# yeyupiaoling/PPASR

Hardware: AMD Instinct MI355X
Metric: audio-seconds/s (RTF^-1) Conformer-streaming fbank, batch32 per GPU, ctc_greedy (higher is better)
Workload: dtype f32; 1 GPU; configs[1]: Conformer streaming (configs/conformer.yml), fbank-80, 32 x 10 s utterances per GPU, V=4233, ctc_greedy, features resident in HBM -> token ids + scores on device; global_batch=32, frames=1000, decoder=ctc_greedy, parallelism=utterance-dp1, pipelined=False, gemm=f32

## Files before the change

### ppasr_amd/csrc/front_fused.hip

```cpp
#include <utility>

#include "conformer_kernels.h"
#include "launch.h"

namespace ppasr {

namespace {
constexpr int kGroupRow[5] = {2, 0, 1, 4, 3};
constexpr int kTapCol[5] = {2, 0, 1, 4, 3};
constexpr int kFactor[5] = {2, 0, 1, 3, 1};
constexpr int quad_slab(int t) { return 4 * kFactor[t / 5] + kFactor[t % 5]; }
constexpr int quad_target(int t) {
  const int g = t / 5, k = t % 5;
  if (g == 0) return k == 0 ? 4 : k <= 2 ? 5 : 4;
  const int a = (g == 1 || g == 2) ? 0 : 2;
  return k == 0 ? (a == 0 ? 5 : 4) : k <= 2 ? a : a + 1;
}
constexpr int quad_fold_src(int t) {
  return t == 1 || t == 5 || t == 21 || t == 23 ? 4 : t == 3 || t == 11 || t == 13 ? 5 : -1;
}
constexpr int quad_fold_mask(int t) {
  return t == 1 ? 0xf : t == 3 ? 0x5 : t == 5 ? 0xa : t == 11 ? 0x2 : t == 13 ? 0x1 : t == 21 ? 0x8 : t == 23 ? 0x4 : 0;
}
constexpr bool quad_fold_clear(int t) { return t == 1 || t == 3 || t == 5 || t == 13 || t == 23; }
static_assert(quad_target(0) == 4 && quad_target(2) == 5 && quad_target(10) == 5 && quad_target(12) == 0 &&
                  quad_target(14) == 1 && quad_target(20) == 4 && quad_target(22) == 2 && quad_target(24) == 3,
              "chunk targets");

template <typename Fn, int... I>
__device__ __forceinline__ void static_for(std::integer_sequence<int, I...>, Fn&& fn) {
  (fn(std::integral_constant<int, I>{}), ...);
}

__host__ __device__ inline int quad_xs_stride(int F, int Q) { return F > 8 * Q + 3 ? F : 8 * Q + 3; }
}

template <bool FROM_Y1>
__device__ __forceinline__ void conv2_quad_body(const float* __restrict__ src, const FrontW& fw, float* __restrict__ out,
                                                int T, int F, int Tp, int F2, int M, int m0, const PadSkip& ps,
                                                const int* __restrict__ tile_tab) {
  constexpr int BP = 32, KC = 128, LD = KC + 4, G = KC / 8, NL = 2, N_CHUNKS = 25;
  constexpr int SLOT = BP * LD;
  const int P = (Tp + 1) >> 1;
  const int Q = (F2 + 1) >> 1;
  int r0 = m0 + blockIdx.x * BP, Mlim = M;
  if (tile_tab) {
    const int t = blockIdx.x, nb = tile_tab[0];
    const int* pre = tile_tab + 1;
    if (t >= pre[nb]) return;
    int lo = 0, hi = nb;
    while (hi - lo > 1) {
      const int mid = (lo + hi) >> 1;
      if (pre[mid] <= t) lo = mid;
      else hi = mid;
    }
    const int S = ps.Tp * ps.unit;
    r0 = lo * S + (t - pre[lo]) * BP;
    Mlim = min(M, (lo + 1) * S);
  } else if (pad_block_skippable(ps, r0, BP, M)) {
    return;
  }
  extern __shared__ __attribute__((aligned(16))) float smem[];
  float* const slot0 = smem;
  float* const slot1 = smem + SLOT;
  f32x4* const y2s = reinterpret_cast<f32x4*>(smem + 2 * SLOT);
  float* const w1s = smem + 2 * SLOT + 5 * NL * 4 * kThreads;
  float* const xs = w1s + 10 * 256;
  const int tid = threadIdx.x, lane = lane_id(), wave = wave_id();
  constexpr int tile_stride = 2 * 16 * G * 64;
  const f32x4* wbase = fw.conv2_wp + (size_t)wave * tile_stride;
  auto seg = [&](int h, int slab) { return wbase + (size_t)(16 * h + slab) * G * 64; };
  BRing<1> ring;
  ring_prime(ring, seg(0, quad_slab(0)), 0);
  const int c4 = tid & 31, rbase = tid >> 5;
  const int bp0 = r0 / Q;
  const int FX = quad_xs_stride(F, Q);
  uint32_t pb = 0;
  int yrow[FROM_Y1 ? NL : 1], yp4[FROM_Y1 ? NL : 1], yq4[FROM_Y1 ? NL : 1];
  if constexpr (!FROM_Y1) {
    for (int idx = tid; idx < 10 * 256; idx += kThreads) w1s[idx] = idx < 9 * 256 ? fw.conv1_w[idx] : fw.conv1_b[idx - 9 * 256];
    const int nbp = (min(r0 + BP, Mlim) - 1) / Q - bp0 + 1;
    for (int idx = tid; idx < nbp * 11 * FX; idx += kThreads) {
      const int fr_row = idx / FX, f = idx - fr_row * FX;
      const int bpl = fr_row / 11, fr = fr_row - 11 * bpl;
      const int bp = bp0 + bpl, b = bp / P, p = bp - b * P;
      const int t = min(8 * p + fr, T - 1);
      xs[idx] = f < F ? (src[((size_t)b * T + t) * F + f] - fw.cmvn_mean[f]) * fw.cmvn_istd[f] : 0.f;
    }
#pragma unroll
    for (int i = 0; i < NL; ++i) {
      const int m = r0 + rbase + 16 * i;
      const int bp = m / Q, q = m - bp * Q;
      const uint32_t v = m < Mlim ? (uint32_t)((bp - bp0) * 11 * FX + 8 * q) : 0xffffu;
      pb |= v << (16 * i);
    }
  } else {
#pragma unroll
    for (int i = 0; i < NL; ++i) {
      const int m = r0 + rbase + 16 * i;
      const int bp = m / Q, q = m - bp * Q, b = bp / P, p = bp - b * P;
      yrow[i] = b * T + 4 * p;
      yp4[i] = 4 * p;
      yq4[i] = m < Mlim ? 4 * q : -1;
    }
  }
  auto pbase = [&](int i) { return (int)((pb >> (16 * i)) & 0xffffu); };
  const int lds_off0 = rbase * LD + 4 * c4;
  float xv[9];
  f32x4 wv[3], bv, ya, yv;
  auto y1_step = [&](int i, int h, int r, int c, int step) {
    const int cc = h * 128 + 4 * c4;
    if constexpr (!FROM_Y1) {
      if (step == 0) {
        const int o = pbase(i);
        const float* p = xs + (o == 0xffff ? 0 : o) + 2 * r * FX + 2 * c;
#pragma unroll
        for (int ii = 0; ii < 3; ++ii)
#pragma unroll
          for (int jj = 0; jj < 3; ++jj) xv[ii * 3 + jj] = p[ii * FX + jj];
        ya = f32x4{0.f, 0.f, 0.f, 0.f};
      } else {
#pragma unroll
        for (int j = 3 * (step - 1); j < 3 * step; ++j)
#pragma unroll
          for (int e = 0; e < 4; ++e) ya[e] = fmaf(wv[j % 3][e], xv[j], ya[e]);
        if (step == 3) {
          ya += bv;
#pragma unroll
          for (int e = 0; e < 4; ++e) ya[e] = pbase(i) != 0xffff ? fmaxf(ya[e], 0.f) : 0.f;
        }
      }
      if (step < 3) {
#pragma unroll
        for (int j = 0; j < 3; ++j) wv[j] = *reinterpret_cast<const f32x4*>(w1s + (3 * step + j) * 256 + cc);
        if (step == 2) bv = *reinterpret_cast<const f32x4*>(w1s + 9 * 256 + cc);
      }
    } else {
      if (step == 0) {
        yv = f32x4{0.f, 0.f, 0.f, 0.f};
        if (yq4[i] >= 0 && yp4[i] + r < T && yq4[i] + c < F)
          yv = *reinterpret_cast<const f32x4*>(src + ((size_t)(yrow[i] + r) * F + yq4[i] + c) * 256 + cc);
      } else if (step == 3) {
        ya = yv;
      }
    }
  };
  auto put = [&](float* buf, int i, const f32x4& v) { *reinterpret_cast<f32x4*>(buf + lds_off0 + i * 16 * LD) = v; };
  auto y2row = [&](int c, int i) -> f32x4& { return y2s[(c * NL + i) * kThreads + tid]; };
  f32x4 z2[NL];
  auto build = [&](auto nc, int g, int h, float* buf) {
    constexpr int n = decltype(nc)::value, grp = n / 5, k = n % 5, r = kGroupRow[grp], c = kTapCol[k];
    const int i = g >> 2, step = g & 3;
    y1_step(i, h, r, c, step);
    if (step != 3) return;
    f32x4 v = ya;
    if constexpr (grp == 0) y2row(c, i) = ya;
    if constexpr (grp == 1 || grp == 3) v = ya - y2row(c, i);
    if constexpr (k == 0) {
      z2[i] = v;
      put(buf, i, v);
    } else if constexpr (k == 1 || k == 3) {
      put(buf, i, v - z2[i]);
    } else {
      put(buf, i, v);
    }
  };
  f32x16 acc[6][1][1];
#pragma unroll
  for (int a = 0; a < 6; ++a) acc_zero(acc[a]);
  auto fold = [&](auto tc, int g) {
    constexpr int t = decltype(tc)::value, fs = quad_fold_src(t), mask = quad_fold_mask(t);
    if constexpr (fs >= 0) {
      const int j = g - 4 * NL;
      int seen = 0;
#pragma unroll
      for (int o = 0; o < 4; ++o) {
        if (!((mask >> o) & 1)) continue;
        if (seen++ == j) {
#pragma unroll
          for (int e = 0; e < 16; ++e) asm volatile("v_add_f32 %0, %0, %1" : "+v"(acc[o][0][0][e]) : "v"(acc[fs][0][0][e]));
        }
      }
      if (quad_fold_clear(t) && j == 4) acc_zero(acc[fs]);
    }
  };
  __syncthreads();
#pragma unroll
  for (int g = 0; g < 4 * NL; ++g) {
    build(std::integral_constant<int, 0>{}, g, 0, slot0);
    __builtin_amdgcn_sched_barrier(0);
  }
  __syncthreads();
  for (int h = 0; h < 2; ++h) {
    asm volatile("" : "+s"(wbase));
    if constexpr (!FROM_Y1) {
      asm volatile("" : "+v"(pb));
    } else {
#pragma unroll
      for (int i = 0; i < NL; ++i) asm volatile("" : "+v"(yrow[i]), "+v"(yp4[i]), "+v"(yq4[i]));
    }
    static_for(std::make_integer_sequence<int, N_CHUNKS>{}, [&](auto tc) {
      constexpr int t = decltype(tc)::value;
      float* const cur = ((t + h) & 1) ? slot1 : slot0;
      float* const nxb = ((t + h) & 1) ? slot0 : slot1;
      const f32x4* nseg = t + 1 < N_CHUNKS ? seg(h, quad_slab(t + 1)) : (h == 0 ? seg(1, quad_slab(0)) : nullptr);
      auto side = [&](int g) {
        if (g < 4 * NL) {
          if constexpr (t + 1 < N_CHUNKS) build(std::integral_constant<int, t + 1>{}, g, h, nxb);
          else if (h == 0) build(std::integral_constant<int, 0>{}, g, 1, nxb);
        } else {
          fold(tc, g);
        }
      };
      rb_gemm<1, 1, G, kPF, decltype(side)>(cur, LD, seg(h, quad_slab(t)), 0, nseg, 0, ring, acc[quad_target(t)], side);
      __syncthreads();
    });
  }
  const int col = wave * 32 + (lane & 31);
  const float b2 = fw.conv2_b[col];
#pragma unroll
  for (int r = 0; r < 16; ++r) {
    const int m = r0 + acc_row(r, lane);
    if (m >= Mlim) continue;
    const int bp = m / Q, q = m - bp * Q, b = bp / P, t0 = 2 * (bp - b * P), f0 = 2 * q;
    float* o = out + ((size_t)(b * Tp + t0) * F2 + f0) * 256 + col;
    const bool f1 = f0 + 1 < F2, t1 = t0 + 1 < Tp;
    o[0] = fmaxf(acc[0][0][0][r] + b2, 0.f);
    if (f1) o[256] = fmaxf(acc[1][0][0][r] + b2, 0.f);
    if (t1) o[(size_t)F2 * 256] = fmaxf(acc[2][0][0][r] + b2, 0.f);
    if (t1 && f1) o[(size_t)F2 * 256 + 256] = fmaxf(acc[3][0][0][r] + b2, 0.f);
  }
}

__global__ __launch_bounds__(kThreads) void k_conv12(const float* __restrict__ feats, FrontW fw, float* __restrict__ out,
                                                     int T, int F, int Tp, int F2, int M, int m0, PadSkip ps,
                                                     const int* __restrict__ tile_tab) {
  conv2_quad_body<false>(feats, fw, out, T, F, Tp, F2, M, m0, ps, tile_tab);
}
__global__ __launch_bounds__(kThreads) void k_conv2_pair(const float* __restrict__ y1, FrontW fw, float* __restrict__ out,
                                                         int T1, int F1, int Tp, int F2, int M, int m0, PadSkip ps,
                                                         const int* __restrict__ tile_tab) {
  conv2_quad_body<true>(y1, fw, out, T1, F1, Tp, F2, M, m0, ps, tile_tab);
}

static int quad_tile_pairs(int Q) { return 31 / Q + 2; }
static size_t quad_lds(bool fused, int F, int F2) {
  const int Q = (F2 + 1) / 2;
  return ((size_t)2 * 32 * 132 + (size_t)5 * 2 * 4 * 512 + (fused ? (size_t)10 * 256 + (size_t)quad_tile_pairs(Q) * 11 * quad_xs_stride(F, Q) : 0)) *
         sizeof(float);
}
bool conv2_quad_supported(const FrontW& fw) { return fw.conv2_wp && fw.conv2_k == 3 && fw.conv2_s == 2; }
bool conv12_supported(const FrontW& fw, int F, int F2) {
  const int Q = (F2 + 1) / 2;
  return conv2_quad_supported(fw) && F2 >= 1 && quad_lds(true, F, F2) <= 160 * 1024 &&
         (size_t)quad_tile_pairs(Q) * 11 * quad_xs_stride(F, Q) < 0xffff;
}

void launch_tile_prefix(const PadSkip& ps, int B, int BM, int* tab, hipStream_t st);

static void launch_quad(bool fused, const float* src, const FrontW& fw, float* y2, int B, int T, int F, int Tp, int F2,
                        hipStream_t st, const PadSkip& ps_frames, int* tile_scratch) {
  const int P = (Tp + 1) / 2, Q = (F2 + 1) / 2;
  PadSkip ps = ps_frames;
  ps.Tp = P;
  ps.mul = 2 * ps_frames.mul;
  ps.slack = (ps_frames.slack + 1) / 2;
  ps.unit = Q;
  const int M = B * P * Q;
  const int* no_tab = nullptr;
#define QUAD(GRID, TAB)                                                                                                  \
  do {                                                                                                                 \
    if (fused)                                                                                                         \
      PPASR_LAUNCH(k_conv12, dim3(GRID), dim3(kThreads), quad_lds(true, F, F2), st, src, fw, y2, T, F, Tp, F2, M, 0, ps, \
                   TAB);                                                                                               \
    else                                                                                                               \
      PPASR_LAUNCH(k_conv2_pair, dim3(GRID), dim3(kThreads), quad_lds(false, F, F2), st, src, fw, y2, T, F, Tp, F2, M, 0, \
                   ps, TAB);                                                                                           \
  } while (0)
  if (ps.lens && tile_scratch) {
    launch_tile_prefix(ps, B, 32, tile_scratch, st);
    QUAD(B * ((P * Q + 31) / 32), (const int*)tile_scratch);
    return;
  }
  QUAD((M + 31) / 32, no_tab);
#undef QUAD
}

void launch_conv12(const float* feats, const FrontW& fw, float* y2, int B, int T, int F, int Tp, int F2, hipStream_t st,
                   const PadSkip& ps_frames, int* tile_scratch) {
  launch_quad(true, feats, fw, y2, B, T, F, Tp, F2, st, ps_frames, tile_scratch);
}
void launch_conv2_quad(const float* y1, const FrontW& fw, float* y2, int B, int T1, int F1, int Tp, int F2, hipStream_t st,
                       const PadSkip& ps_frames, int* tile_scratch) {
  launch_quad(false, y1, fw, y2, B, T1, F1, Tp, F2, st, ps_frames, tile_scratch);
}

hipError_t configure_front_fused_kernels() {
  hipError_t e;
#define SET_LDS(fn)                                                                                              \
  e = hipFuncSetAttribute(reinterpret_cast<const void*>(fn), hipFuncAttributeMaxDynamicSharedMemorySize, 160 * 1024); \
  if (e != hipSuccess) return e;
  SET_LDS(k_conv12);
  SET_LDS(k_conv2_pair);
#undef SET_LDS
  return hipSuccess;
}

}
```

Measured before the change: 58430 audio-s/s.

## Compute conv1 im2col tile with MFMA 32x32x2 instead of scalar FMAs

In the fused front-end conv kernel, the first 3x3 convolution (conv1) on the CMVN-normalized fbank tile was computed with per-thread scalar FMAs. It is now computed by the first four waves using chains of mfma_f32_32x32x2f32. The bias is folded in as a fifth K pair through a constant-one input, with ReLU applied through inline v_max. Precomputed LDS byte offsets replace the packed per-row base, and the out-of-range rows read a zeroed tail region. This moves conv1 arithmetic off the VALU so it can overlap the conv2 GEMM pipeline. In exchange it adds hand-placed s_nop hazard padding and a different lane-to-row mapping that must stay consistent with the LDS layout.

```diff
diff --git a/ppasr_amd/csrc/front_fused.hip b/ppasr_amd/csrc/front_fused.hip
--- a/ppasr_amd/csrc/front_fused.hip
+++ b/ppasr_amd/csrc/front_fused.hip
@@ -30,6 +30,12 @@
 template <typename Fn, int... I>
 __device__ __forceinline__ void static_for(std::integer_sequence<int, I...>, Fn&& fn) {
   (fn(std::integral_constant<int, I>{}), ...);
+}
+
+__device__ __forceinline__ float relu1(float x) {
+  float d;
+  asm("v_max_f32 %0, 0, %1" : "=v"(d) : "v"(x));
+  return d;
 }
 
 __host__ __device__ inline int quad_xs_stride(int F, int Q) { return F > 8 * Q + 3 ? F : 8 * Q + 3; }
@@ -75,8 +81,10 @@
   const int c4 = tid & 31, rbase = tid >> 5;
   const int bp0 = r0 / Q;
   const int FX = quad_xs_stride(F, Q);
-  uint32_t pb = 0;
+  const int hh = lane >> 5;
   int yrow[FROM_Y1 ? NL : 1], yp4[FROM_Y1 ? NL : 1], yq4[FROM_Y1 ? NL : 1];
+  uint32_t xoff[5] = {0, 0, 0, 0, 0};
+  float one = 0.f;
   if constexpr (!FROM_Y1) {
     for (int idx = tid; idx < 10 * 256; idx += kThreads) w1s[idx] = idx < 9 * 256 ? fw.conv1_w[idx] : fw.conv1_b[idx - 9 * 256];
     const int nbp = (min(r0 + BP, Mlim) - 1) / Q - bp0 + 1;
@@ -87,12 +95,17 @@
       const int t = min(8 * p + fr, T - 1);
       xs[idx] = f < F ? (src[((size_t)b * T + t) * F + f] - fw.cmvn_mean[f]) * fw.cmvn_istd[f] : 0.f;
     }
-#pragma unroll
-    for (int i = 0; i < NL; ++i) {
-      const int m = r0 + rbase + 16 * i;
-      const int bp = m / Q, q = m - bp * Q;
-      const uint32_t v = m < Mlim ? (uint32_t)((bp - bp0) * 11 * FX + 8 * q) : 0xffffu;
-      pb |= v << (16 * i);
+    if (r0 + BP > Mlim)
+      for (int idx = tid; idx < 11 * FX; idx += kThreads) xs[nbp * 11 * FX + idx] = 0.f;
+    const int m = r0 + (lane & 31);
+    const int bp = m / Q, q = m - bp * Q;
+    const bool live = m < Mlim;
+    const int base = (int)(xs - smem) + (live ? (bp - bp0) * 11 * FX + 8 * q : nbp * 11 * FX);
+    one = live ? 1.f : 0.f;
+#pragma unroll
+    for (int mm = 0; mm < 5; ++mm) {
+      const int j = min(2 * mm + hh, 8);
+      xoff[mm] = (uint32_t)(base + (j / 3) * FX + j % 3) * 4u;
     }
   } else {
 #pragma unroll
@@ -104,51 +117,22 @@
       yq4[i] = m < Mlim ? 4 * q : -1;
     }
   }
-  auto pbase = [&](int i) { return (int)((pb >> (16 * i)) & 0xffffu); };
   const int lds_off0 = rbase * LD + 4 * c4;
-  float xv[9];
-  f32x4 wv[3], bv, ya, yv;
+  f32x4 ya, yv;
   auto y1_step = [&](int i, int h, int r, int c, int step) {
     const int cc = h * 128 + 4 * c4;
-    if constexpr (!FROM_Y1) {
-      if (step == 0) {
-        const int o = pbase(i);
-        const float* p = xs + (o == 0xffff ? 0 : o) + 2 * r * FX + 2 * c;
-#pragma unroll
-        for (int ii = 0; ii < 3; ++ii)
-#pragma unroll
-          for (int jj = 0; jj < 3; ++jj) xv[ii * 3 + jj] = p[ii * FX + jj];
-        ya = f32x4{0.f, 0.f, 0.f, 0.f};
-      } else {
-#pragma unroll
-        for (int j = 3 * (step - 1); j < 3 * step; ++j)
-#pragma unroll
-          for (int e = 0; e < 4; ++e) ya[e] = fmaf(wv[j % 3][e], xv[j], ya[e]);
-        if (step == 3) {
-          ya += bv;
-#pragma unroll
-          for (int e = 0; e < 4; ++e) ya[e] = pbase(i) != 0xffff ? fmaxf(ya[e], 0.f) : 0.f;
-        }
-      }
-      if (step < 3) {
-#pragma unroll
-        for (int j = 0; j < 3; ++j) wv[j] = *reinterpret_cast<const f32x4*>(w1s + (3 * step + j) * 256 + cc);
-        if (step == 2) bv = *reinterpret_cast<const f32x4*>(w1s + 9 * 256 + cc);
-      }
-    } else {
-      if (step == 0) {
-        yv = f32x4{0.f, 0.f, 0.f, 0.f};
-        if (yq4[i] >= 0 && yp4[i] + r < T && yq4[i] + c < F)
-          yv = *reinterpret_cast<const f32x4*>(src + ((size_t)(yrow[i] + r) * F + yq4[i] + c) * 256 + cc);
-      } else if (step == 3) {
-        ya = yv;
-      }
+    if (step == 0) {
+      yv = f32x4{0.f, 0.f, 0.f, 0.f};
+      if (yq4[i] >= 0 && yp4[i] + r < T && yq4[i] + c < F)
+        yv = *reinterpret_cast<const f32x4*>(src + ((size_t)(yrow[i] + r) * F + yq4[i] + c) * 256 + cc);
+    } else if (step == 3) {
+      ya = yv;
     }
   };
   auto put = [&](float* buf, int i, const f32x4& v) { *reinterpret_cast<f32x4*>(buf + lds_off0 + i * 16 * LD) = v; };
   auto y2row = [&](int c, int i) -> f32x4& { return y2s[(c * NL + i) * kThreads + tid]; };
   f32x4 z2[NL];
-  auto build = [&](auto nc, int g, int h, float* buf) {
+  auto build_twin = [&](auto nc, int g, int h, float* buf) {
     constexpr int n = decltype(nc)::value, grp = n / 5, k = n % 5, r = kGroupRow[grp], c = kTapCol[k];
     const int i = g >> 2, step = g & 3;
     y1_step(i, h, r, c, step);
@@ -165,6 +149,55 @@
       put(buf, i, v);
     }
   };
+  float w1a[5] = {0.f, 0.f, 0.f, 0.f, 0.f};
+  auto load_w1 = [&](int h) {
+    if (wave >= 4) return;
+#pragma unroll
+    for (int mm = 0; mm < 5; ++mm) w1a[mm] = w1s[(2 * mm + hh) * 256 + h * 128 + 32 * wave + (lane & 31)];
+  };
+  float xw[5];
+  f32x16 y1t;
+  f32x4 zc[4], d1v;
+  const int lds_row0 = (lane & 31) * LD + 32 * (wave & 3) + 4 * hh;
+  auto d1row = [&](int c, int qd) -> f32x4& { return y2s[(c * 4 + qd) * 256 + (tid & 255)]; };
+  auto build_mfma = [&](auto nc, int g, float* buf) {
+    constexpr int n = decltype(nc)::value, grp = n / 5, k = n % 5, r = kGroupRow[grp], c = kTapCol[k];
+    if (wave >= 4) return;
+    if (g == 0) {
+      const uint32_t pos = (uint32_t)(2 * r * FX + 2 * c) * 4u;
+#pragma unroll
+      for (int mm = 0; mm < 5; ++mm)
+        xw[mm] = *reinterpret_cast<const float*>(reinterpret_cast<const char*>(smem) + (xoff[mm] + pos));
+    } else if (g == 1 || g == 2) {
+      if (g == 1) {
+        xw[4] = hh ? one : xw[4];
+        const f32x16 zero = {0.f, 0.f, 0.f, 0.f, 0.f, 0.f, 0.f, 0.f, 0.f, 0.f, 0.f, 0.f, 0.f, 0.f, 0.f, 0.f};
+        y1t = __builtin_amdgcn_mfma_f32_32x32x2f32(w1a[0], xw[0], zero, 0, 0, 0);
+        y1t = __builtin_amdgcn_mfma_f32_32x32x2f32(w1a[1], xw[1], y1t, 0, 0, 0);
+        y1t = __builtin_amdgcn_mfma_f32_32x32x2f32(w1a[2], xw[2], y1t, 0, 0, 0);
+      } else {
+        y1t = __builtin_amdgcn_mfma_f32_32x32x2f32(w1a[3], xw[3], y1t, 0, 0, 0);
+        y1t = __builtin_amdgcn_mfma_f32_32x32x2f32(w1a[4], xw[4], y1t, 0, 0, 0);
+      }
+    }
+    if (g >= 4) {
+      const int qd = g - 4;
+      f32x4 v;
+#pragma unroll
+      for (int e = 0; e < 4; ++e) v[e] = relu1(y1t[4 * qd + e]);
+      if constexpr (grp == 0) d1row(c, qd) = v;
+      if constexpr (grp == 1 || grp == 3) v = v - d1v;
+      if constexpr (k == 0) zc[qd] = v;
+      if constexpr (k == 1 || k == 3) v = v - zc[qd];
+      *reinterpret_cast<f32x4*>(buf + lds_row0 + 8 * qd) = v;
+    }
+    if constexpr (grp == 1 || grp == 3)
+      if (g >= 3 && g < 7) d1v = d1row(c, g - 3);
+  };
+  auto build = [&](auto nc, int g, int h, float* buf) {
+    if constexpr (FROM_Y1) build_twin(nc, g, h, buf);
+    else build_mfma(nc, g, buf);
+  };
   f32x16 acc[6][1][1];
 #pragma unroll
   for (int a = 0; a < 6; ++a) acc_zero(acc[a]);
@@ -185,16 +218,20 @@
     }
   };
   __syncthreads();
+  if constexpr (!FROM_Y1) load_w1(0);
 #pragma unroll
   for (int g = 0; g < 4 * NL; ++g) {
     build(std::integral_constant<int, 0>{}, g, 0, slot0);
+    if constexpr (!FROM_Y1)
+      if (g == 3) asm volatile("s_nop 7\n\ts_nop 7\n\ts_nop 3");
     __builtin_amdgcn_sched_barrier(0);
   }
   __syncthreads();
   for (int h = 0; h < 2; ++h) {
     asm volatile("" : "+s"(wbase));
     if constexpr (!FROM_Y1) {
-      asm volatile("" : "+v"(pb));
+#pragma unroll
+      for (int mm = 0; mm < 5; ++mm) asm volatile("" : "+v"(xoff[mm]));
     } else {
 #pragma unroll
       for (int i = 0; i < NL; ++i) asm volatile("" : "+v"(yrow[i]), "+v"(yp4[i]), "+v"(yq4[i]));
@@ -207,7 +244,11 @@
       auto side = [&](int g) {
         if (g < 4 * NL) {
           if constexpr (t + 1 < N_CHUNKS) build(std::integral_constant<int, t + 1>{}, g, h, nxb);
-          else if (h == 0) build(std::integral_constant<int, 0>{}, g, 1, nxb);
+          else if (h == 0) {
+            if constexpr (!FROM_Y1)
+              if (g == 0) load_w1(1);
+            build(std::integral_constant<int, 0>{}, g, 1, nxb);
+          }
         } else {
           fold(tc, g);
         }
```

Result: no change. 58620 audio-s/s (median of 6 runs) (+0.3%).
